# adria0/plonk-by-fingers

Measured on AMD Instinct MI355X. Metric: NTT elements/sec (Goldilocks, n=2^20 per GPU, natural order, bit-exact vs src/fft.rs), higher is better.
Workload: dtype u64 (Goldilocks p=2^64-2^32+1); 1 GPU; Goldilocks forward NTT, batch 32 x 2^20; n_per_gpu=1048576, n_global=1048576, batch=32, passes=default (2^20: 10,10)

## Files before the change

### plonk-by-fingers_amd/csrc/ntt_gl.hpp

```cpp
#pragma once
#include "ntt_kernels.hpp"

namespace pbf {

struct GlPassArgs {
  const uint64_t* in;
  uint64_t* out;
  const uint64_t* twpass;
  const uint64_t* tw0;
  const uint64_t* tw1;
  const uint64_t* tc;
  const uint64_t* tws_a;
  const uint64_t* tws_b;
  uint64_t n;
  uint32_t log_n;
  uint32_t log_ns;
  uint32_t tw_bits;
  uint32_t blocks_per_poly;
  uint32_t batch;
  uint32_t scaled;
  uint32_t out_split_log;
  uint32_t xcd_kmajor;
  uint64_t in_pitch, out_pitch;
  const uint64_t* post_tw;
  uint32_t skip_pass_tw;
  uint64_t blk_pitch;
  const uint64_t* cs_tab;
  const uint64_t* cs_tab1;
  uint32_t cs_bits;
  uint64_t cs_len;
};

__host__ __device__ constexpr bool gl_pow2_neg(int k) {
  const int raw = ((k % 192) + 192) % 192;
  return raw > 64 && raw <= 160;
}
template <int K>
__device__ __forceinline__ uint64_t gl_pow2_abs(uint64_t x) {
  constexpr int RAW = ((K % 192) + 192) % 192;
  if constexpr (RAW == 0) {
    return x;
  } else if constexpr (RAW > 160) {
    return gl_div_pow2<192 - RAW>(x);
  } else {
    using T = ShiftKind<RAW>;
    static_assert(T::NEG == gl_pow2_neg(K), "sign of 2^K");
    return apply_shift<Goldilocks, T>(x);
  }
}
template <int K>
__device__ __forceinline__ uint64_t gl_pow2(uint64_t x) {
  const uint64_t y = gl_pow2_abs<K>(x);
  if constexpr (gl_pow2_neg(K)) {
    const FieldArgs f{};
    return Goldilocks::sub(0, y, f);
  } else {
    return y;
  }
}

template <int E64, int Q1, int S2 = 1>
__device__ __forceinline__ void gl_stage_b_twiddle(uint64_t* v) {
  if constexpr (S2 < 16) {
    v[S2] = gl_pow2<(E64 * S2 * Q1) % 192>(v[S2]);
    gl_stage_b_twiddle<E64, Q1, S2 + 1>(v);
  }
}
template <int E64, int Q1, int S2 = 1>
__device__ __forceinline__ void gl_stage_b_twiddle_abs(uint64_t* v) {
  if constexpr (S2 < 16) {
    v[S2] = gl_pow2_abs<(E64 * S2 * Q1) % 192>(v[S2]);
    gl_stage_b_twiddle_abs<E64, Q1, S2 + 1>(v);
  }
}
__host__ __device__ constexpr unsigned gl_stage_b_negmask(int e64, int q1) {
  unsigned m = 0;
  for (int s2 = 1; s2 < 16; ++s2) m |= gl_pow2_neg((e64 * s2 * q1) % 192) ? 1u << s2 : 0u;
  return m;
}
constexpr int GL_B_LEVELS = 2;
template <int E64, int Q1>
__device__ __forceinline__ void gl_stage_b_head(uint64_t* v) {
  const FieldArgs f{};
  gl_stage_b_twiddle_abs<E64, Q1>(v);
  dft_reg_signed<Goldilocks, 4, sub_root_exp(E64, 4), gl_stage_b_negmask(E64, Q1), GL_B_LEVELS>(v, f);
}

template <int E64, int Q, int E = 1>
__device__ __forceinline__ void gl_post_twiddle_br(uint64_t* v) {
  if constexpr (E < 16) {
    v[bitrev_c(E, 4)] = gl_pow2<(E64 * E * Q) % 192>(v[bitrev_c(E, 4)]);
    gl_post_twiddle_br<E64, Q, E + 1>(v);
  }
}
template <int E64, int WV, int U = 0>
__device__ __forceinline__ void gl_rg3_c_shift(uint64_t* x) {
  if constexpr (U < 4) {
    constexpr int g = WV + 4 * U;
    x[U * 4 + 1] = gl_pow2<(E64 * g) % 192>(x[U * 4 + 1]);
    x[U * 4 + 2] = gl_pow2<(E64 * 2 * g) % 192>(x[U * 4 + 2]);
    x[U * 4 + 3] = gl_pow2<(E64 * 3 * g) % 192>(x[U * 4 + 3]);
    gl_rg3_c_shift<E64, WV, U + 1>(x);
  }
}

template <int LOGR, int TILE>
struct GlShape {
  static constexpr int R = 1 << LOGR;
  static constexpr int LOGC = LOGR - 6;
  static constexpr int C = 1 << LOGC;
  static constexpr int W = TILE / R;
  static constexpr int NT = TILE / 16;
  static constexpr int WPQ = NT / 256;
  static constexpr bool YX = W == 16 && C > 1;
  static constexpr int YP = (YX ? 64 : 65) * W;
  static constexpr int LDS = (C * YP > TILE) ? C * YP : TILE;
  static constexpr bool LDS32K = LDS * 8 <= 32768;
  static constexpr int NSUB_C = (64 * W) / NT;
  __host__ __device__ static constexpr int ysw(int k1) {
    return W <= 32 ? (k1 / (32 / W)) & (W - 1) : (k1 & 31);
  }
  __host__ __device__ static constexpr int yidx(int r2, int k1, int w) {
    return r2 * YP + (YX ? (k1 ^ (r2 & 1)) : k1) * W + (w ^ ysw(k1));
  }
};

__device__ __forceinline__ void gl_tile_coords(const GlPassArgs& a, uint32_t tile, uint32_t tiles, uint32_t* poly,
                                               uint32_t* kb) {
  if (a.xcd_kmajor == 1) {
    const uint32_t v = (tile & 7) * (tiles >> 3) + (tile >> 3);
    *kb = v / a.batch;
    *poly = v % a.batch;
  } else if (a.xcd_kmajor == 2) {
    const uint32_t v = (tile & 7) * (tiles >> 3) + (tile >> 3);
    *poly = v / a.blocks_per_poly;
    *kb = v % a.blocks_per_poly;
  } else {
    *poly = tile / a.blocks_per_poly;
    *kb = tile % a.blocks_per_poly;
  }
}

__device__ __forceinline__ uint64_t gl_cs_factor(const GlPassArgs& a, uint64_t i) {
  const FieldArgs f{};
  if (a.cs_tab1) return Goldilocks::mul(a.cs_tab[i & ((1ull << a.cs_bits) - 1)], a.cs_tab1[i >> a.cs_bits], f);
  return a.cs_tab[i];
}

constexpr int GL_STORES = 16;

constexpr uint64_t GL_BLK_PITCH = 8192;
static_assert(GL_BLK_PITCH >= 8192 && GL_BLK_PITCH % 2 == 0, "block pitch");
typedef uint64_t gl_u64x2 __attribute__((ext_vector_type(2)));

template <int LOGR, int E64, bool FIRST, int TILE, int RG = 0, int CS = 0, int SP = 0>
__device__ __forceinline__ void gl_tile(const GlPassArgs& a, uint64_t* lds, uint32_t tile, uint32_t tiles, int t) {
  using Sh = GlShape<LOGR, TILE>;
  constexpr int C = Sh::C, LOGC = Sh::LOGC, W = Sh::W, NT = Sh::NT, YP = Sh::YP;
  (void)YP;
  static_assert(Sh::NSUB_C * C == GL_STORES, "stores per thread");
  static_assert(SP == 0 || ((!FIRST || SP == 2) && RG == 0 && CS == 0 && SP <= 2), "SP: plain two-pass plan");
  static_assert(SP != 2 || (LOGR == 10 && TILE == 8192), "SP 2: the 10,10 plan");
  static_assert(RG == 0 || (LOGR == 8 && TILE == 4096 && FIRST == (RG == 1)), "RG shape");
  static_assert(CS == 0 || (FIRST == (CS == 1) && (RG == 0 || RG == 2 * CS - 1)), "CS 1: first pass, CS 2: last pass");
  const FieldArgs f{};
  using G = Goldilocks;
  uint32_t poly, kb;
  gl_tile_coords(a, tile, tiles, &poly, &kb);
  const uint64_t j0 = (uint64_t)kb * W;
  const uint64_t* in = a.in + (uint64_t)poly * a.in_pitch;
  const uint64_t stride = a.n >> LOGR;
  constexpr bool BLK_IN = SP == 2 && !FIRST, BLK_OUT = SP == 2 && FIRST;

  uint64_t v[16];
  if constexpr (BLK_IN) {
    const gl_u64x2* blk = (const gl_u64x2*)(in + (uint64_t)kb * a.blk_pitch) + t;
#pragma unroll
    for (int up = 0; up < 8; ++up) {
      const gl_u64x2 e = blk[512 * up];
      v[(2 * (up & 1)) * 4 + (up >> 1)] = e.x;
      v[(2 * (up & 1) + 1) * 4 + (up >> 1)] = e.y;
    }
  } else if constexpr (CS == 1) {
#pragma unroll
    for (int h = 0; h < 2; ++h) {
      uint64_t tw[8];
#pragma unroll
      for (int uu = 0; uu < 2; ++uu) {
        const int idx = t + NT * (2 * h + uu);
        const int w = idx % W, r2 = (idx / W) % C, s2 = idx / (C * W);
#pragma unroll
        for (int s1 = 0; s1 < 4; ++s1) {
          const uint64_t i = (j0 + w) + (uint64_t)(16 * C * s1 + C * s2 + r2) * stride;
          const bool on = i < a.cs_len;
          v[8 * h + uu * 4 + s1] = on ? in[i] : 0;
          tw[uu * 4 + s1] = on ? gl_cs_factor(a, i) : 0;
        }
      }
#pragma unroll
      for (int m = 0; m < 8; ++m) v[8 * h + m] = G::mul(v[8 * h + m], tw[m], f);
    }
  } else {
#pragma unroll
    for (int u = 0; u < 4; ++u) {
      const int idx = t + NT * u;
      const int w = idx % W, r2 = (idx / W) % C, s2 = idx / (C * W);
#pragma unroll
      for (int s1 = 0; s1 < 4; ++s1) {
        const int r = 16 * C * s1 + C * s2 + r2;
        v[u * 4 + s1] = in[(j0 + w) + (uint64_t)r * stride];
      }
    }
  }
  uint64_t t3[RG == 3 ? 2 : 1];
  if constexpr (RG == 3) {
    const int wave = t >> 6, q1 = wave / Sh::WPQ, rw = (wave % Sh::WPQ) * 64 + (t & 63);
    const int r2 = rw / W, w = rw % W;
    const uint64_t X = ((uint64_t)q1 << 16) + j0 + w;
    t3[0] = a.tws_a[((uint64_t)r2 << 18) + X];
    t3[1] = a.tws_b[X];
  }
  if constexpr (!FIRST && RG != 3 && SP == 0) if (!a.skip_pass_tw) {
    const uint64_t kmask = (1ull << a.log_ns) - 1;
#pragma unroll
    for (int h = 0; h < 2; ++h) {
      uint64_t tw[8];
#pragma unroll
      for (int uu = 0; uu < 2; ++uu) {
        const int u = 2 * h + uu;
        const int idx = t + NT * u;
        const int w = idx % W, r2 = (idx / W) % C, s2 = idx / (C * W);
        const uint64_t k = (j0 + w) & kmask;
#pragma unroll
        for (int s1 = 0; s1 < 4; ++s1) {
          const uint64_t r = (uint64_t)(16 * C * s1 + C * s2 + r2);
          if (a.twpass) {
            tw[uu * 4 + s1] = a.twpass[(r << a.log_ns) + k];
          } else if (a.tws_a) {
            tw[uu * 4 + s1] = G::mul(a.tws_b[(uint64_t)kb * Sh::R + r], a.tws_a[r * W + w], f);
          } else {
            const uint64_t e = ((r * k) << (a.log_n - a.log_ns - LOGR)) & (a.n - 1);
            tw[uu * 4 + s1] = G::mul(a.tw0[e & ((1ull << a.tw_bits) - 1)], a.tw1[e >> a.tw_bits], f);
          }
        }
      }
#pragma unroll
      for (int m = 0; m < 8; ++m) v[8 * h + m] = G::mul(v[8 * h + m], tw[m], f);
    }
  }
#pragma unroll
  for (int u = 0; u < 4; ++u) dft_reg<G, 2, sub_root_exp(E64, 2)>(v + u * 4, nullptr, f);
  if constexpr (BLK_IN) {
#pragma unroll
    for (int h = 0; h < 2; ++h) {
      const int s2 = 8 * h + (t >> 6);
#pragma unroll
      for (int q1 = 0; q1 < 4; ++q1) {
        gl_u64x2 e;
        e.x = v[(2 * h) * 4 + bitrev_c(q1, 2)];
        e.y = v[(2 * h + 1) * 4 + bitrev_c(q1, 2)];
        *(gl_u64x2*)(lds + (q1 * 16 + s2) * (C * W) + 2 * (t & 63)) = e;
      }
    }
  } else {
#pragma unroll
    for (int u = 0; u < 4; ++u) {
      const int idx = t + NT * u;
      const int s2 = idx / (C * W), rw = idx % (C * W);
#pragma unroll
      for (int q1 = 0; q1 < 4; ++q1) lds[(q1 * 16 + s2) * (C * W) + rw] = v[u * 4 + bitrev_c(q1, 2)];
    }
  }
  __syncthreads();

  {
    const int wave = t >> 6;
    const int q1 = wave / Sh::WPQ;
    const int rw = (wave % Sh::WPQ) * 64 + (t & 63);
#pragma unroll
    for (int s2 = 0; s2 < 16; ++s2) v[s2] = lds[(q1 * 16 + s2) * (C * W) + rw];
    if constexpr (RG == 3) {
      uint64_t p = t3[0];
      const uint64_t d = t3[1];
#pragma unroll
      for (int s2 = 0; s2 < 16; ++s2) {
        v[s2] = G::mul(v[s2], p, f);
        if (s2 < 15) p = G::mul(p, d, f);
      }
      dft_reg<G, 4, sub_root_exp(E64, 4)>(v, nullptr, f);
    } else {
      switch (__builtin_amdgcn_readfirstlane(q1)) {
        case 1: gl_stage_b_head<E64, 1>(v); break;
        case 2: gl_stage_b_head<E64, 2>(v); break;
        case 3: gl_stage_b_head<E64, 3>(v); break;
        default: gl_stage_b_head<E64, 0>(v); break;
      }
      dft_reg_tail<G, 4, sub_root_exp(E64, 4), GL_B_LEVELS>(v, f);
    }
    __syncthreads();
    const int r2 = rw / W, w = rw % W;
#pragma unroll
    for (int q2 = 0; q2 < 16; ++q2) {
      const int k1 = q1 + 4 * q2;
      lds[Sh::yidx(r2, k1, w)] = v[bitrev_c(q2, 4)];
    }
  }
  __syncthreads();

  auto c_map = [&](int u, int* k1, int* w) {
    const int idx = t + NT * u;
    if constexpr (BLK_OUT) {
      *k1 = 8 * (t >> 6) + (t & 7);
      *w = (t >> 3) & 7;
    } else if constexpr (FIRST) {
      *k1 = idx & 63;
      *w = idx >> 6;
    } else {
      *k1 = idx / W;
      *w = idx % W;
    }
  };
  uint64_t x[Sh::NSUB_C * C];
#pragma unroll
  for (int u = 0; u < Sh::NSUB_C; ++u) {
    int k1, w;
    c_map(u, &k1, &w);
#pragma unroll
    for (int r2 = 0; r2 < C; ++r2) x[u * C + r2] = lds[Sh::yidx(r2, k1, w)];
  }
  if constexpr (RG == 3) {
    switch (__builtin_amdgcn_readfirstlane(t >> 6)) {
      case 0: gl_rg3_c_shift<E64, 0>(x); break;
      case 1: gl_rg3_c_shift<E64, 1>(x); break;
      case 2: gl_rg3_c_shift<E64, 2>(x); break;
      default: gl_rg3_c_shift<E64, 3>(x); break;
    }
  } else if constexpr (RG == 1) {
    const uint64_t* tc = a.tc + ((j0 >> 12) & 15) * 256;
#pragma unroll
    for (int u = 0; u < Sh::NSUB_C; ++u) {
      int k1, w;
      c_map(u, &k1, &w);
      uint64_t tw[C];
#pragma unroll
      for (int r2 = 0; r2 < C; ++r2) tw[r2] = tc[r2 * 64 + k1];
#pragma unroll
      for (int r2 = 0; r2 < C; ++r2) x[u * C + r2] = G::mul(x[u * C + r2], tw[r2], f);
    }
  } else {
    uint64_t tw[Sh::NSUB_C * C];
    const bool scaled = SP == 0 && a.scaled;
    const int r2lo = scaled ? 0 : 1;
#pragma unroll
    for (int u = 0; u < Sh::NSUB_C; ++u) {
      int k1, w;
      c_map(u, &k1, &w);
#pragma unroll
      for (int r2 = 0; r2 < C; ++r2) tw[u * C + r2] = (r2 >= r2lo) ? a.tc[r2 * 64 + k1] : 1;
    }
    if (scaled) {
#pragma unroll
      for (int m = 0; m < Sh::NSUB_C * C; ++m) x[m] = G::mul(x[m], tw[m], f);
    } else {
#pragma unroll
      for (int u = 0; u < Sh::NSUB_C; ++u)
#pragma unroll
        for (int r2 = 1; r2 < C; ++r2) x[u * C + r2] = G::mul(x[u * C + r2], tw[u * C + r2], f);
    }
  }
  if constexpr (C > 1) {
#pragma unroll
    for (int u = 0; u < Sh::NSUB_C; ++u) dft_reg<G, LOGC, sub_root_exp(E64, LOGC)>(x + u * C, nullptr, f);
  }

  if constexpr (BLK_OUT) {
    static_assert(Sh::NSUB_C == 1 && W == 8, "tile-major stores: one sub-DFT per thread");
    const uint64_t base = (uint64_t)__builtin_amdgcn_readfirstlane(t >> 6) * a.blk_pitch + j0 * W;
    const uint32_t lane = t & 63;
    const uint64_t* ptw = a.post_tw + base;
    uint64_t* o = a.out + (uint64_t)poly * a.out_pitch + base;
    uint64_t tw[C];
#pragma unroll
    for (int k2 = 0; k2 < C; ++k2) tw[k2] = ptw[(uint64_t)(8 * k2) * a.blk_pitch + lane];
#pragma unroll
    for (int k2 = 0; k2 < C; ++k2) x[bitrev_c(k2, LOGC)] = G::mul(x[bitrev_c(k2, LOGC)], tw[k2], f);
#pragma unroll
    for (int k2 = 0; k2 < C; ++k2) o[(uint64_t)(8 * k2) * a.blk_pitch + lane] = x[bitrev_c(k2, LOGC)];
  } else if constexpr (FIRST) {
    uint64_t* o = a.out + (uint64_t)poly * a.out_pitch;
#pragma unroll
    for (int u = 0; u < Sh::NSUB_C; ++u) {
      int k1, w;
      c_map(u, &k1, &w);
      const uint64_t base = (j0 + w) << LOGR;
      if (a.post_tw) {
        uint64_t tw[C];
#pragma unroll
        for (int k2 = 0; k2 < C; ++k2) tw[k2] = a.post_tw[base + k1 + 64 * k2];
#pragma unroll
        for (int k2 = 0; k2 < C; ++k2) x[u * C + bitrev_c(k2, LOGC)] = G::mul(x[u * C + bitrev_c(k2, LOGC)], tw[k2], f);
      }
#pragma unroll
      for (int k2 = 0; k2 < C; ++k2) o[base + k1 + 64 * k2] = x[u * C + bitrev_c(k2, LOGC)];
    }
  } else {
    const uint32_t lns = SP == 2 ? (uint32_t)LOGR : a.log_ns;
    const uint64_t ns_mask = (1ull << lns) - 1;
    uint64_t* out = a.out + (uint64_t)poly * a.out_pitch;
    const uint32_t sl = SP != 0 ? 0u : a.out_split_log;
#pragma unroll
    for (int u = 0; u < Sh::NSUB_C; ++u) {
      int k1, w;
      c_map(u, &k1, &w);
      const uint64_t j = j0 + w;
      const uint64_t base = ((j >> lns) << (lns + LOGR)) + (j & ns_mask);
      if (sl == 0) {
        if constexpr (CS == 2) {
          uint64_t tw[C];
#pragma unroll
          for (int k2 = 0; k2 < C; ++k2) tw[k2] = gl_cs_factor(a, base + ((uint64_t)(k1 + 64 * k2) << lns));
#pragma unroll
          for (int k2 = 0; k2 < C; ++k2) x[u * C + bitrev_c(k2, LOGC)] = G::mul(x[u * C + bitrev_c(k2, LOGC)], tw[k2], f);
        }
#pragma unroll
        for (int k2 = 0; k2 < C; ++k2) out[base + ((uint64_t)(k1 + 64 * k2) << lns)] = x[u * C + bitrev_c(k2, LOGC)];
      } else {
        const uint64_t smask = (1ull << sl) - 1;
#pragma unroll
        for (int k2 = 0; k2 < C; ++k2) {
          const uint64_t kk = base + ((uint64_t)(k1 + 64 * k2) << lns);
          a.out[((((kk >> sl) * a.batch) + poly) << sl) + (kk & smask)] = x[u * C + bitrev_c(k2, LOGC)];
        }
      }
    }
  }
}

template <int LOGR, int TILE>
__device__ __forceinline__ void gl_shape_checks() {
  using Sh = GlShape<LOGR, TILE>;
  static_assert(LOGR >= 6 && LOGR <= 10, "radix 2^6 .. 2^10");
  static_assert(Sh::LDS * 8 <= (TILE > 8192 ? 160 : 80) * 1024, "LDS budget");
  static_assert(Sh::W >= 8 && Sh::WPQ >= 1, "tile shape");
}

template <int LOGR, int E64, bool FIRST, int TILE, int RG = 0, int CS = 0, int SP = 0>
__global__ void __launch_bounds__(TILE / 16)
__attribute__((amdgpu_waves_per_eu((FIRST || RG) && GlShape<LOGR, TILE>::LDS32K ? 5 : 4)))
ntt_gl_pass_kernel(GlPassArgs a) {
  gl_shape_checks<LOGR, TILE>();
  __shared__ __attribute__((aligned(16))) uint64_t lds[GlShape<LOGR, TILE>::LDS];
  const uint32_t tiles = a.blocks_per_poly * a.batch;
  gl_tile<LOGR, E64, FIRST, TILE, RG, CS, SP>(a, lds, blockIdx.x, tiles, threadIdx.x);
}

template <int E64>
__global__ void __launch_bounds__(256) __attribute__((amdgpu_waves_per_eu(4))) ntt_gl_rg2_kernel(GlPassArgs a) {
  constexpr int W = 16;
  __shared__ __attribute__((aligned(16))) uint64_t lds[16 * 16 * W];
  const FieldArgs f{};
  using G = Goldilocks;
  const uint32_t tiles = a.blocks_per_poly * a.batch;
  uint32_t poly, kb;
  gl_tile_coords(a, blockIdx.x, tiles, &poly, &kb);
  const int t = threadIdx.x, w = t % W, a1h = t / W;
  const uint64_t j0 = (uint64_t)kb * W, j = j0 + w;
  const uint32_t c = (uint32_t)(j0 >> 6) & 3, a1l = (uint32_t)(j0 >> 14) & 3;
  const uint64_t* in = a.in + (uint64_t)poly * a.in_pitch;
  const uint64_t stride = a.n >> 8;
  uint64_t v[16], tw[16];
#pragma unroll
  for (int a2l = 0; a2l < 16; ++a2l) v[a2l] = in[j + (uint64_t)(a2l * 16 + a1h) * stride];
  const uint64_t* t2 = a.twpass + ((uint64_t)(a1l + 4 * a1h) << 12) + (j & 255);
#pragma unroll
  for (int d = 0; d < 16; ++d) tw[d] = t2[256 * d];
  switch (__builtin_amdgcn_readfirstlane(c)) {
    case 1: gl_stage_b_twiddle<E64, 1>(v); break;
    case 2: gl_stage_b_twiddle<E64, 2>(v); break;
    case 3: gl_stage_b_twiddle<E64, 3>(v); break;
    default: break;
  }
  dft_reg<G, 4, sub_root_exp(E64, 4)>(v, nullptr, f);
#pragma unroll
  for (int d = 0; d < 16; ++d) lds[d * 256 + (a1h ^ (d & 3)) * W + w] = G::mul(v[bitrev_c(d, 4)], tw[d], f);
  __syncthreads();
  const int d2 = t / W;
#pragma unroll
  for (int h = 0; h < 16; ++h) v[h] = lds[d2 * 256 + (h ^ (d2 & 3)) * W + w];
  dft_reg<G, 4, sub_root_exp(E64, 4)>(v, nullptr, f);
  switch (__builtin_amdgcn_readfirstlane(a1l)) {
    case 1: gl_post_twiddle_br<E64, 1>(v); break;
    case 2: gl_post_twiddle_br<E64, 2>(v); break;
    case 3: gl_post_twiddle_br<E64, 3>(v); break;
    default: break;
  }
  uint64_t* out = a.out + (uint64_t)poly * a.out_pitch;
  const uint64_t base = ((j >> 8) << 16) + (j & 255);
#pragma unroll
  for (int e = 0; e < 16; ++e) out[base + ((uint64_t)(d2 + 16 * e) << 8)] = v[bitrev_c(e, 4)];
}

}
```

### plonk-by-fingers_amd/csrc/ntt_launch.hip

```cpp
#include <cstdlib>
#include <cstring>
#include <mutex>
#include "internal.hpp"
#include "ntt_gl.hpp"

namespace pbf {

bool hinv(uint64_t a, uint64_t m, uint64_t* out) {
  __int128 s = 0, old_s = 1, r = m, old_r = a % m;
  while (r != 0) {
    __int128 q = old_r / r, t;
    t = old_r - q * r; old_r = r; r = t;
    t = old_s - q * s; old_s = s; s = t;
  }
  if (old_r != 1) return false;
  if (old_s < 0) old_s += m;
  *out = (uint64_t)old_s;
  return true;
}

bool field_for(uint64_t m, FieldKind* kind, FieldArgs* fa) {
  fa->m = m;
  fa->mu = 0;
  if (m == GOLDILOCKS) { *kind = FIELD_GOLDILOCKS; return true; }
// ... 241 lines not shown
  if (rc) return rc;
  if ((rc = run_plan_impl(p, d_in, (uint64_t*)s2.p, batch, s0, s1, stream, 0))) return rc;
  hipLaunchKernelGGL(shard_split_kernel, dim3(grid_for(p.n * batch)), dim3(256), 0, stream, (const uint64_t*)s2.p,
                     d_send, S, p.n, (uint32_t)batch);
  PBF_HIP(hipGetLastError());
  return 0;
}

int launch_shard_unsplit(const uint64_t* recv, uint64_t* out, uint64_t nl, uint32_t batch, uint32_t G,
                         hipStream_t s) {
  hipLaunchKernelGGL(shard_unsplit_kernel, dim3(grid_for(nl * batch)), dim3(256), 0, s, recv, out, nl / G, nl, batch,
                     G);
  PBF_HIP(hipGetLastError());
  return 0;
}

int make_two_level(uint64_t m, uint64_t root, uint64_t n, TwoLevel* t) {
  uint32_t log_n = 0;
  while ((1ull << log_n) < n) ++log_n;
  t->bits = (log_n + 1) / 2;
  t->root = root;
  const auto tw = two_level_tabs(root, n, t->bits, 1, m);
  int rc = upload(t->t0, tw.first);
  return rc ? rc : upload(t->t1, tw.second);
}

template <class F>
static int combine_typed(const FieldArgs& fa, const TwoLevel& tl, uint32_t G, uint64_t rank, const uint64_t* in,
                         uint64_t* out, uint64_t nl, uint32_t batch, int inverse, hipStream_t s) {
  CombineArgs a;
  a.recv = in; a.out = out;
  a.tw0 = (const uint64_t*)tl.t0.p; a.tw1 = (const uint64_t*)tl.t1.p; a.tw_bits = tl.bits;
  a.nl = nl; a.s = nl / G; a.rank = rank; a.n_mask = (uint64_t)G * nl - 1; a.batch = batch; a.f = fa;
  a.scale = 1;
  if (inverse) {
    uint64_t ginv;
    if (!hinv(G % fa.m, fa.m, &ginv)) return fail(2, "G has no inverse");
    a.scale = ginv;
  }
  for (int i = 0; i < 8; ++i) a.wg[i] = 0;
  const uint64_t wG = hpow(tl.root, nl, fa.m);
  uint64_t x = 1 % fa.m;
  for (uint32_t i = 0; i < G; ++i) { a.wg[i] = x; x = hmul(x, wG, fa.m); }
  const uint64_t total = (nl / G) * batch;
  void (*fn)(CombineArgs) = nullptr;
  switch (G) {
    case 2: fn = inverse ? shard_split_inv_kernel<F, 2> : shard_combine_kernel<F, 2>; break;
    case 4: fn = inverse ? shard_split_inv_kernel<F, 4> : shard_combine_kernel<F, 4>; break;
    case 8: fn = inverse ? shard_split_inv_kernel<F, 8> : shard_combine_kernel<F, 8>; break;
    default: return fail(1, "world size must be 2, 4 or 8");
  }
  hipLaunchKernelGGL(fn, dim3(grid_for(total)), dim3(256), 0, s, a);
  PBF_HIP(hipGetLastError());
  return 0;
}

int launch_shard_combine(FieldKind k, const FieldArgs& fa, const TwoLevel& tl, uint32_t G, uint64_t rank,
                         const uint64_t* in, uint64_t* out, uint64_t nl, uint32_t batch, int inverse, hipStream_t s) {
  return with_field(k, [&](auto F) {
    return combine_typed<decltype(F)>(fa, tl, G, rank, in, out, nl, batch, inverse, s);
  });
}

typedef void (*GlPassFn)(GlPassArgs);

struct GlPassDesc {
  int logr;
  bool first;
  int rg;
  int cs;
  int sp;
};

static bool two_pass_tw(const NttPlan& p, uint32_t split_log) {
  return p.logr.size() == 2 && split_log == 0 && p.twpass[1]->p;
}

static bool gl_blocked(const NttPlan& p, bool coset, uint32_t split_log) {
  return two_pass_tw(p, split_log) && !coset && p.post_blk.p != nullptr;
}

static uint64_t gl_scratch_pitch(const NttPlan& p, bool coset, uint32_t split_log) {
  return gl_blocked(p, coset, split_log) ? 128 * GL_BLK_PITCH : p.n;
}

static GlPassDesc gl_pass_desc(const NttPlan& p, size_t i, bool coset, uint32_t split_log) {
  const size_t P = p.logr.size();
  GlPassDesc d{p.logr[i], i == 0, 0, 0, 0};
  if (p.rg && P == 3 && split_log == 0) d.rg = (int)i + 1;
  if (coset && !p.inverse && i == 0) d.cs = 1;
  if (coset && p.inverse && i == P - 1) d.cs = 2;
  if (gl_blocked(p, coset, split_log)) d.sp = 2;
  else if (two_pass_tw(p, split_log) && i == 1 && !coset && !p.inverse && p.e64 == 39 && d.logr == 10) d.sp = 1;
  return d;
}

template <int E, int LR>
static GlPassFn gl_kernel_lr(const GlPassDesc& d) {
  constexpr int T = gl_tile(LR);
  if (d.first) return d.cs ? ntt_gl_pass_kernel<LR, E, true, T, 0, 1> : ntt_gl_pass_kernel<LR, E, true, T>;
  return d.cs ? ntt_gl_pass_kernel<LR, E, false, T, 0, 2> : ntt_gl_pass_kernel<LR, E, false, T>;
}

template <int E>
static GlPassFn gl_kernel_e(const GlPassDesc& d) {
  if (d.rg == 1) return d.cs ? ntt_gl_pass_kernel<8, E, true, 4096, 1, 1> : ntt_gl_pass_kernel<8, E, true, 4096, 1>;
  if (d.rg == 2) return ntt_gl_rg2_kernel<E>;
  if (d.rg == 3) return d.cs ? ntt_gl_pass_kernel<8, E, false, 4096, 3, 2> : ntt_gl_pass_kernel<8, E, false, 4096, 3>;
  if constexpr (E == 39) {
    if (d.sp == 1) return ntt_gl_pass_kernel<10, E, false, 8192, 0, 0, 1>;
    if (d.sp == 2) return d.first ? ntt_gl_pass_kernel<10, E, true, 8192, 0, 0, 2> : ntt_gl_pass_kernel<10, E, false, 8192, 0, 0, 2>;
  }
  switch (d.logr) {
    case 6: return gl_kernel_lr<E, 6>(d);
    case 7: return gl_kernel_lr<E, 7>(d);
    case 8: return gl_kernel_lr<E, 8>(d);
    case 9: return gl_kernel_lr<E, 9>(d);
    case 10: return gl_kernel_lr<E, 10>(d);
    default: return nullptr;
  }
}

static GlPassFn gl_kernel(const GlPassDesc& d, int e64) {
  return e64 == 39 ? gl_kernel_e<39>(d) : gl_kernel_e<153>(d);
}

static int run_gl_group(const NttPlan& p, const uint64_t* d_in, uint64_t* d_out, size_t batch, DevBuf& s0,
                        DevBuf& s1, hipStream_t stream, uint32_t split_log, size_t soff = 0,
                        const GlCoset* cs = nullptr);

int ForkSet::ensure(int streams) {
  if (streams > GL_MAX_STREAMS) streams = GL_MAX_STREAMS;
  const unsigned flags = hipEventDisableTiming | hipEventDisableSystemFence;
  if (streams > 1 && !fork) PBF_HIP(hipEventCreateWithFlags(&fork, flags));
  for (int i = 1; i < streams; ++i) {
    if (!aux[i]) PBF_HIP(hipStreamCreateWithFlags(&aux[i], hipStreamNonBlocking));
    if (!join[i]) PBF_HIP(hipEventCreateWithFlags(&join[i], flags));
  }
  return 0;
}

ForkSet::~ForkSet() {
  (void)hipSetDevice(device);
  for (int i = 1; i < GL_MAX_STREAMS; ++i) {
    if (aux[i]) {
      (void)hipStreamSynchronize(aux[i]);
      (void)hipStreamDestroy(aux[i]);
    }
    if (join[i]) (void)hipEventDestroy(join[i]);
  }
  if (fork) (void)hipEventDestroy(fork);
}

static void gl_schedule(const NttPlan& p, size_t batch, uint32_t split_log, const ForkSet* fork, size_t* G, int* ns) {
  const long long go = p.opts.num("ntt.group", -1);
  *G = go >= 0 ? (size_t)go : (batch >= 8 ? 4 : batch);
  if (split_log != 0 || *G >= batch) *G = 0;
  *ns = (int)p.opts.num("ntt.streams", 2);
  *ns = *ns < 1 ? 1 : (*ns > GL_MAX_STREAMS ? GL_MAX_STREAMS : *ns);
  if (!fork || *G == 0) *ns = 1;
}

static size_t gl_scratch_polys(const NttPlan& p, size_t batch, uint32_t split_log, const ForkSet* fork) {
  size_t G;
  int ns;
  gl_schedule(p, batch, split_log, fork, &G, &ns);
  return (G == 0 || G * ns > batch) ? batch : G * ns;
}

static int run_gl_passes(const NttPlan& p, const uint64_t* d_in, uint64_t* d_out, size_t batch, DevBuf& s0,
                         DevBuf& s1, hipStream_t stream, uint32_t split_log, ForkSet* fork, const GlCoset* cs) {
  size_t G;
  int ns;
  gl_schedule(p, batch, split_log, fork, &G, &ns);
  if (G == 0) return run_gl_group(p, d_in, d_out, batch, s0, s1, stream, split_log, 0, cs);
  const size_t in_pitch = (cs && !p.inverse) ? cs->in_len : p.n;
  hipStream_t sts[GL_MAX_STREAMS];
  sts[0] = stream;
  if (ns > 1) {
    int rc = fork->ensure(ns);
    if (rc) return rc;
    for (int i = 1; i < ns; ++i) sts[i] = fork->aux[i];
    PBF_HIP(hipEventRecord(fork->fork, stream));
    for (int i = 1; i < ns; ++i) PBF_HIP(hipStreamWaitEvent(sts[i], fork->fork, 0));
  }
  int gi = 0;
  for (size_t g0 = 0; g0 < batch; g0 += G, ++gi) {
    const size_t b = batch - g0 < G ? batch - g0 : G;
    const int rc = run_gl_group(p, d_in + g0 * in_pitch, d_out + g0 * p.n, b, s0, s1, sts[gi % ns], 0,
                                (size_t)(gi % ns) * G * gl_scratch_pitch(p, cs != nullptr, split_log), cs);
    if (rc) return rc;
  }
  for (int i = 1; i < ns; ++i) {
    PBF_HIP(hipEventRecord(fork->join[i], sts[i]));
    PBF_HIP(hipStreamWaitEvent(stream, fork->join[i], 0));
  }
  return 0;
}

static int ensure_rg_tables(const NttPlan& p) {
  if (p.rg_built) return 0;
  const uint64_t m = p.m, n = p.n;
  const uint64_t w = p.root;
  int rc;
  const uint64_t w4096 = hpow(w, n / 4096, m);
  std::vector<uint64_t> tc1(4096);
  for (uint64_t a2l = 0; a2l < 16; ++a2l)
    for (uint64_t r2 = 0; r2 < 4; ++r2)
      for (uint64_t k1 = 0; k1 < 64; ++k1)
        tc1[a2l * 256 + r2 * 64 + k1] = hpow(w4096, ((a2l + 16 * r2) * k1) % 4096, m);
  const Table t2 = pass_tab(hpow(w, 64, m), 64, 4096, m);
  const uint64_t scale = p.inverse ? p.n_inv : 1;
  std::vector<uint64_t> tgc(4ull << 18), tgb(1ull << 18);
  {
    const uint64_t w4 = hpow(w, 4, m);
    uint64_t x1 = 1, x4 = 1;
    for (uint64_t X = 0; X < (1ull << 18); ++X) {
      tgb[X] = x4;
      uint64_t c = scale;
      for (uint64_t r2 = 0; r2 < 4; ++r2) {
        tgc[(r2 << 18) + X] = c;
        c = hmul(c, x1, m);
      }
      x1 = hmul(x1, w, m);
      x4 = hmul(x4, w4, m);
    }
  }
  if ((rc = upload(p.rg_tc1, tc1)) || (rc = upload(p.rg_t2, t2)) || (rc = upload(p.rg_tgc, tgc)) ||
      (rc = upload(p.rg_tgb, tgb)))
    return rc;
  p.rg_built = true;
  return 0;
}

static GlPassArgs gl_pass_args(const NttPlan& p, size_t i, const GlPassDesc& d, uint32_t log_ns, const uint64_t* in,
                               uint64_t* out, size_t batch, uint32_t split_log, const GlCoset* cs) {
  const bool last = i == p.logr.size() - 1;
  const uint64_t W = (uint64_t)gl_tile(d.logr) >> d.logr;
  GlPassArgs a;
  a.in = in;
  a.out = out;
  a.in_pitch = a.out_pitch = p.n;
  a.twpass = (const uint64_t*)p.twpass[i]->p;
  a.tw0 = (const uint64_t*)p.tw0.p;
  a.tw1 = (const uint64_t*)p.tw1.p;
  a.tc = (const uint64_t*)p.tc[i]->p;
  const bool tws = !a.twpass && last && p.tws_a && (uint64_t)p.tws_w == W;
  a.tws_a = tws ? (const uint64_t*)p.tws_a->p : nullptr;
  a.tws_b = tws ? (const uint64_t*)p.tws_b->p : nullptr;
  a.n = p.n;
  a.log_n = p.log_n;
  a.log_ns = log_ns;
  a.tw_bits = p.tw_bits;
  a.blocks_per_poly = (uint32_t)((p.n >> d.logr) / W);
  a.batch = (uint32_t)batch;
  a.scaled = (p.inverse && last) ? 1 : 0;
  a.out_split_log = last ? split_log : 0;
  const uint64_t tiles = (uint64_t)a.blocks_per_poly * batch;
  a.xcd_kmajor = (log_ns > 0 && batch > 1 && tiles % 8 == 0) ? 1 : 0;
  a.post_tw = nullptr;
  a.skip_pass_tw = 0;
  if (two_pass_tw(p, split_log)) {
    if (i == 0) a.post_tw = (const uint64_t*)p.twpass[1]->p;
    else a.skip_pass_tw = 1;
  }
  if (a.post_tw && batch > 1 && tiles % 8 == 0) a.xcd_kmajor = 1;
  a.blk_pitch = 0;
  if (d.sp == 2) {
    a.blk_pitch = GL_BLK_PITCH;
    if (i == 0) {
      a.post_tw = (const uint64_t*)p.post_blk.p;
      a.out_pitch = 128 * GL_BLK_PITCH;
    } else {
      a.in_pitch = 128 * GL_BLK_PITCH;
      a.xcd_kmajor = 0;
    }
  }
  a.cs_tab = a.cs_tab1 = nullptr;
  a.cs_bits = 0;
  a.cs_len = 0;
  if (d.cs) {
    a.cs_tab = (const uint64_t*)cs->tabs->t0.p;
    a.cs_tab1 = (const uint64_t*)cs->tabs->t1.p;
    a.cs_bits = cs->tabs->bits;
    if (d.cs == 1) {
      a.cs_len = cs->in_len;
      a.in_pitch = cs->in_len;
    } else if (!d.rg) {
      a.tc = (const uint64_t*)cs->tabs->tc_last.p;
      a.scaled = 0;
    }
  }
  if (d.rg) {
    if (d.rg == 1) a.tc = (const uint64_t*)p.rg_tc1.p;
    if (d.rg == 2) a.twpass = (const uint64_t*)p.rg_t2.p;
    if (d.rg == 3) {
      a.twpass = nullptr;
      a.tws_a = (const uint64_t*)p.rg_tgc.p;
      a.tws_b = (const uint64_t*)p.rg_tgb.p;
    }
    if (tiles % 8 == 0) a.xcd_kmajor = 2;
  }
  return a;
}

static int run_gl_group(const NttPlan& p, const uint64_t* d_in, uint64_t* d_out, size_t batch, DevBuf& s0,
                        DevBuf& s1, hipStream_t stream, uint32_t split_log, size_t soff, const GlCoset* cs) {
  const size_t P = p.logr.size();
  if (cs && (split_log != 0 || P < 2)) return fail(1, "coset transform: unsupported plan");
  if (gl_pass_desc(p, 0, cs != nullptr, split_log).rg) {
    const int rc = ensure_rg_tables(p);
    if (rc) return rc;
  }
  uint32_t log_ns = 0;
  for (size_t i = 0; i < P; ++i) {
    const GlPassDesc d = gl_pass_desc(p, i, cs != nullptr, split_log);
    const GlPassFn fn = gl_kernel(d, p.e64);
    if (!fn) return fail(1, "no Goldilocks pass kernel for this radix");
    const int tile = gl_tile(d.logr);
    if ((p.n >> d.logr) % (tile >> d.logr)) return fail(1, "transform too small for the pass tile");
    const uint64_t* in = (i == 0) ? d_in : (const uint64_t*)(((i - 1) & 1) ? s1.p : s0.p) + soff;
    uint64_t* out = (i == P - 1) ? d_out : (uint64_t*)((i & 1) ? s1.p : s0.p) + soff;
    const GlPassArgs a = gl_pass_args(p, i, d, log_ns, in, out, batch, split_log, cs);
    const uint64_t tiles = (uint64_t)a.blocks_per_poly * batch;
    if (tiles > 0x7fffffffull) return fail(1, "batch too large");
    hipLaunchKernelGGL(fn, dim3((uint32_t)tiles), dim3(tile / 16), 0, stream, a);
    PBF_HIP(hipGetLastError());
    log_ns += d.logr;
  }
  return 0;
}

static int run_plan_impl(const NttPlan& p, const uint64_t* d_in, uint64_t* d_out, size_t batch, DevBuf& s0,
                         DevBuf& s1, hipStream_t stream, uint32_t split_log, ForkSet* fork, const GlCoset* cs) {
  if (batch == 0) return 0;
  if (p.n == 1) {
    if (d_in != d_out) PBF_HIP(hipMemcpyAsync(d_out, d_in, batch * 8, hipMemcpyDeviceToDevice, stream));
    return 0;
  }
  if (p.logr.empty()) {
    with_field(p.kind, [&](auto F) {
      hipLaunchKernelGGL(ntt_small_kernel<decltype(F)>, dim3(batch), dim3(256), 0, stream, d_in, d_out,
                         (const uint64_t*)p.small_tw.p, p.log_n, p.n_inv, (uint32_t)p.inverse, p.fa);
    });
    PBF_HIP(hipGetLastError());
    return 0;
  }
  const size_t P = p.logr.size();
  const size_t bytes = p.gl ? gl_scratch_polys(p, batch, split_log, fork) * gl_scratch_pitch(p, cs != nullptr, split_log) * 8
                            : batch * p.n * 8;
  int rc = s0.ensure(bytes);
  if (!rc && P > 2) rc = s1.ensure(bytes);
  if (rc) return rc;
  uint32_t log_ns = 0;
  if (p.gl) return run_gl_passes(p, d_in, d_out, batch, s0, s1, stream, split_log, fork, cs);
  if (cs) return fail(1, "coset transform: not a Goldilocks standard-root plan");
  for (size_t i = 0; i < P; ++i) {
    const int lr = p.logr[i];
    const PassFn fn = pass_fn(p.kind, p.e64, lr);
    if (!fn) return fail(1, "no kernel for this radix");
    const int W = cols_for(lr);
    PassArgs a;
    a.in = (i == 0) ? d_in : (const uint64_t*)(((i - 1) & 1) ? s1.p : s0.p);
    a.out = (i == P - 1) ? d_out : (uint64_t*)((i & 1) ? s1.p : s0.p);
    a.tw0 = (const uint64_t*)p.tw0.p;
    a.tw1 = (const uint64_t*)p.tw1.p;
    a.rtab = (const uint64_t*)p.rtab[i]->p;
    a.twpass = (const uint64_t*)p.twpass[i]->p;
    a.n = p.n;
    a.n_inv = p.n_inv;
    a.log_n = p.log_n;
    a.log_ns = log_ns;
    a.tw_bits = p.tw_bits;
    a.blocks_per_poly = (uint32_t)((p.n >> lr) / W);
    a.scale = (p.inverse && i == P - 1) ? 1 : 0;
    a.out_split_log = (i == P - 1) ? split_log : 0;
    a.batch = (uint32_t)batch;
    a.f = p.fa;
    const int nt = (W << lr) >> NTT_LQ;
    const uint64_t blocks = (uint64_t)a.blocks_per_poly * batch;
    if (blocks > 0x7fffffffull) return fail(1, "batch too large");
    const uint32_t grid = (uint32_t)blocks;
    a.xcd_kmajor = (log_ns > 0 && batch > 1 && grid % 8 == 0) ? 1 : 0;
    hipLaunchKernelGGL(fn, dim3(grid), dim3(nt), 0, stream, a);
    PBF_HIP(hipGetLastError());
    log_ns += lr;
  }
  return 0;
}

static uint32_t log2_ceil(uint64_t x) {
  uint32_t l = 0;
  while ((1ull << l) < x) ++l;
  return l;
}

static int coset_tabs(const NttPlan& p, uint64_t shift, uint64_t len, const CosetTabs** out) {
  const uint64_t m = p.m;
  CosetTabs* t = nullptr;
  for (auto& c : p.coset)
    if (c->shift == shift) t = c.get();
  if (t && t->len >= len) {
    t->stamp = ++p.coset_clock;
    *out = t;
    return 0;
  }
  if (!t) {
    if (p.coset.size() >= COSET_SHIFTS_PER_PLAN) {
      size_t old = 0;
      for (size_t i = 1; i < p.coset.size(); ++i)
        if (p.coset[i]->stamp < p.coset[old]->stamp) old = i;
      p.coset.erase(p.coset.begin() + old);
    }
    p.coset.emplace_back(new CosetTabs());
    t = p.coset.back().get();
    t->shift = shift;
  } else {
    PBF_HIP(hipDeviceSynchronize());
  }
  t->len = 0;
  uint64_t s = shift, c = 1 % m;
  if (p.inverse) {
    if (!hinv(shift, m, &s)) return fail(1, "shift has no inverse");
    if (p.gl && !p.rg) c = p.n_inv;
  }
  int rc;
  if (len <= (1ull << p.twmax_log)) {
    t->bits = 0;
    t->t1.release();
    if ((rc = upload(t->t0, geometric(c, s, len, m)))) return rc;
  } else {
    t->bits = (log2_ceil(len) + 1) / 2;
    const auto tw = two_level_tabs(s, len, t->bits, c, m);
    if ((rc = upload(t->t0, tw.first)) || (rc = upload(t->t1, tw.second))) return rc;
  }
  if (p.gl && !p.rg && p.inverse && !t->tc_last.p) {
    const uint64_t R = 1ull << p.logr.back();
    if ((rc = upload(t->tc_last, stage_c_tab(hpow(p.root, p.n / R, m), R / 64, 1, m)))) return rc;
  }
  t->len = len;
  t->stamp = ++p.coset_clock;
  *out = t;
  return 0;
}

template <class F>
__global__ void coset_scale_kernel(const uint64_t* in, uint64_t in_len, uint64_t* out, uint64_t n, uint64_t batch,
                                   const uint64_t* t0, const uint64_t* t1, uint32_t bits, FieldArgs f) {
  const uint64_t total = n * batch;
  for (uint64_t id = (uint64_t)blockIdx.x * blockDim.x + threadIdx.x; id < total;
       id += (uint64_t)gridDim.x * blockDim.x) {
    const uint64_t b = id / n, i = id % n;
    uint64_t y = 0;
    if (i < in_len) {
      const uint64_t tw = t1 ? F::mul(t0[i & ((1ull << bits) - 1)], t1[i >> bits], f) : t0[i];
      y = F::mul(in[b * in_len + i], tw, f);
    }
    out[id] = y;
  }
}

static int launch_coset_scale(const NttPlan& p, const CosetTabs& t, const uint64_t* in, uint64_t in_len, uint64_t* out,
                              uint64_t batch, hipStream_t s) {
  const dim3 grid((uint32_t)grid_for(p.n * batch));
  with_field(p.kind, [&](auto F) {
    hipLaunchKernelGGL(coset_scale_kernel<decltype(F)>, grid, dim3(256), 0, s, in, in_len, out, p.n, batch,
                       (const uint64_t*)t.t0.p, (const uint64_t*)t.t1.p, t.bits, p.fa);
  });
  PBF_HIP(hipGetLastError());
  return 0;
}

int run_plan_coset(const NttPlan& p, uint64_t shift, const uint64_t* d_in, size_t in_len, uint64_t* d_out,
                   size_t batch, DevBuf& s0, DevBuf& s1, hipStream_t stream, ForkSet* fork) {
  if (batch == 0) return 0;
  if (p.n == 1 || (shift == 1 && in_len == p.n)) return run_plan_impl(p, d_in, d_out, batch, s0, s1, stream, 0, fork);
  const CosetTabs* t;
  int rc = coset_tabs(p, shift, p.inverse ? p.n : in_len, &t);
  if (rc) return rc;
  if (p.gl) {
    const GlCoset cs{t, in_len};
    return run_plan_impl(p, d_in, d_out, batch, s0, s1, stream, 0, fork, &cs);
  }
  if (p.inverse) {
    if ((rc = run_plan_impl(p, d_in, d_out, batch, s0, s1, stream, 0, fork))) return rc;
    return launch_coset_scale(p, *t, d_out, p.n, d_out, batch, stream);
  }
  if ((rc = launch_coset_scale(p, *t, d_in, in_len, d_out, batch, stream))) return rc;
  return run_plan_impl(p, d_out, d_out, batch, s0, s1, stream, 0, fork);
}

int launch_pointwise_mul(FieldKind k, const FieldArgs& fa, const uint64_t* a, const uint64_t* b, uint64_t* c,
                         uint64_t count, hipStream_t s) {
  uint64_t blocks = (count + 255) / 256;
  if (blocks > 4096) blocks = 4096;
  if (blocks == 0) return 0;
  with_field(k, [&](auto F) {
    hipLaunchKernelGGL(pointwise_mul_kernel<decltype(F)>, dim3(blocks), dim3(256), 0, s, a, b, c, count, fa);
  });
  PBF_HIP(hipGetLastError());
  return 0;
}
// ... 95 lines not shown
```

Baseline: 112.4 billion elements/s.

## Exchange 64-bit values through LDS in 32-bit halves to fit three workgroups per CU

For the 10,10 blocked plan, the in-tile LDS transposes now move the low and high 32-bit halves of each value in two rounds. This halves the LDS buffer so three workgroups fit per CU, and waves_per_eu is raised to 6. The reads are hand-written ds_read_b32 inline asm with fixed strides. The cost is extra barriers and twice as many LDS instructions. Separately, the default batch group size goes from 4 to 8 for blocked plans when the batch is at least 16.

```diff
diff --git a/plonk-by-fingers_amd/csrc/ntt_gl.hpp b/plonk-by-fingers_amd/csrc/ntt_gl.hpp
--- a/plonk-by-fingers_amd/csrc/ntt_gl.hpp
+++ b/plonk-by-fingers_amd/csrc/ntt_gl.hpp
@@ -149,6 +149,35 @@
 
 constexpr int GL_STORES = 16;
 
+__host__ __device__ constexpr bool gl_split(int sp) { return sp == 2; }
+typedef uint32_t gl_u32x2 __attribute__((ext_vector_type(2)));
+#define GL_RD(i, off) "ds_read_b32 %" #i ", %16 offset:" #off "\n\t"
+template <int STRIDE>
+__device__ __forceinline__ void gl_lds_read16(const uint32_t* p, uint32_t* o) {
+  static_assert(STRIDE == 512 || STRIDE == 2080, "the strides written out below: Z (C*W words), Y (YP words)");
+  const uint32_t a = (uint32_t)(uintptr_t)(const __attribute__((address_space(3))) uint32_t*)p;
+#define GL_RD_OUT                                                                                                   \
+  "=&v"(o[0]), "=&v"(o[1]), "=&v"(o[2]), "=&v"(o[3]), "=&v"(o[4]), "=&v"(o[5]), "=&v"(o[6]), "=&v"(o[7]), "=&v"(o[8]), \
+      "=&v"(o[9]), "=&v"(o[10]), "=&v"(o[11]), "=&v"(o[12]), "=&v"(o[13]), "=&v"(o[14]), "=&v"(o[15])
+  if constexpr (STRIDE == 512) {
+    asm volatile(GL_RD(0, 0) GL_RD(1, 512) GL_RD(2, 1024) GL_RD(3, 1536) GL_RD(4, 2048) GL_RD(5, 2560) GL_RD(6, 3072)
+                     GL_RD(7, 3584) GL_RD(8, 4096) GL_RD(9, 4608) GL_RD(10, 5120) GL_RD(11, 5632) GL_RD(12, 6144)
+                         GL_RD(13, 6656) GL_RD(14, 7168) GL_RD(15, 7680) "s_waitcnt lgkmcnt(0)"
+                 : GL_RD_OUT
+                 : "v"(a)
+                 : "memory");
+  } else {
+    asm volatile(GL_RD(0, 0) GL_RD(1, 2080) GL_RD(2, 4160) GL_RD(3, 6240) GL_RD(4, 8320) GL_RD(5, 10400) GL_RD(6, 12480)
+                     GL_RD(7, 14560) GL_RD(8, 16640) GL_RD(9, 18720) GL_RD(10, 20800) GL_RD(11, 22880) GL_RD(12, 24960)
+                         GL_RD(13, 27040) GL_RD(14, 29120) GL_RD(15, 31200) "s_waitcnt lgkmcnt(0)"
+                 : GL_RD_OUT
+                 : "v"(a)
+                 : "memory");
+  }
+#undef GL_RD_OUT
+}
+#undef GL_RD
+
 constexpr uint64_t GL_BLK_PITCH = 8192;
 static_assert(GL_BLK_PITCH >= 8192 && GL_BLK_PITCH % 2 == 0, "block pitch");
 typedef uint64_t gl_u64x2 __attribute__((ext_vector_type(2)));
@@ -171,6 +200,9 @@
   const uint64_t* in = a.in + (uint64_t)poly * a.in_pitch;
   const uint64_t stride = a.n >> LOGR;
   constexpr bool BLK_IN = SP == 2 && !FIRST, BLK_OUT = SP == 2 && FIRST;
+  constexpr bool SPLIT = gl_split(SP);
+  uint32_t* lds32 = (uint32_t*)lds;
+  (void)lds32;
 
   uint64_t v[16];
   if constexpr (BLK_IN) {
@@ -250,7 +282,46 @@
   }
 #pragma unroll
   for (int u = 0; u < 4; ++u) dft_reg<G, 2, sub_root_exp(E64, 2)>(v + u * 4, nullptr, f);
-  if constexpr (BLK_IN) {
+  if constexpr (SPLIT) {
+    const int q1r = (t >> 6) / Sh::WPQ, rwr = ((t >> 6) % Sh::WPQ) * 64 + (t & 63);
+    uint32_t zl[16];
+#pragma unroll
+    for (int hw = 0; hw < 2; ++hw) {
+      if (hw) __syncthreads();
+      if constexpr (BLK_IN) {
+#pragma unroll
+        for (int h = 0; h < 2; ++h) {
+          const int s2 = 8 * h + (t >> 6);
+#pragma unroll
+          for (int q1 = 0; q1 < 4; ++q1) {
+            gl_u32x2 e;
+            e.x = (uint32_t)(v[(2 * h) * 4 + bitrev_c(q1, 2)] >> (32 * hw));
+            e.y = (uint32_t)(v[(2 * h + 1) * 4 + bitrev_c(q1, 2)] >> (32 * hw));
+            *(gl_u32x2*)(lds32 + (q1 * 16 + s2) * (C * W) + 2 * (t & 63)) = e;
+          }
+        }
+      } else {
+#pragma unroll
+        for (int u = 0; u < 4; ++u) {
+          const int idx = t + NT * u;
+          const int s2 = idx / (C * W), rw = idx % (C * W);
+#pragma unroll
+          for (int q1 = 0; q1 < 4; ++q1)
+            lds32[(q1 * 16 + s2) * (C * W) + rw] = (uint32_t)(v[u * 4 + bitrev_c(q1, 2)] >> (32 * hw));
+        }
+      }
+      __syncthreads();
+      static_assert(C * W * 4 == 512, "Z stride of gl_lds_read16");
+      if (hw == 0) {
+        gl_lds_read16<512>(lds32 + q1r * 16 * (C * W) + rwr, zl);
+      } else {
+        uint32_t zh[16];
+        gl_lds_read16<512>(lds32 + q1r * 16 * (C * W) + rwr, zh);
+#pragma unroll
+        for (int s2 = 0; s2 < 16; ++s2) v[s2] = ((uint64_t)zh[s2] << 32) | zl[s2];
+      }
+    }
+  } else if constexpr (BLK_IN) {
 #pragma unroll
     for (int h = 0; h < 2; ++h) {
       const int s2 = 8 * h + (t >> 6);
@@ -271,14 +342,25 @@
       for (int q1 = 0; q1 < 4; ++q1) lds[(q1 * 16 + s2) * (C * W) + rw] = v[u * 4 + bitrev_c(q1, 2)];
     }
   }
-  __syncthreads();
-
+  if constexpr (!SPLIT) __syncthreads();
+
+  int tc = t;
+  auto y_write_half = [&](int hw) {
+    const int wv = tc >> 6, q1 = wv / Sh::WPQ, rw = (wv % Sh::WPQ) * 64 + (tc & 63);
+    const int r2 = rw / W, w = rw % W;
+    static_assert(!SPLIT || (W == 8 && Sh::yidx(3, 2 + 4 * 13, 6) == 3 * YP + 2 * W + (6 ^ (13 & 7)) + 4 * W * 13), "Y address form");
+#pragma unroll
+    for (int q2 = 0; q2 < 16; ++q2)
+      lds32[(r2 * YP + q1 * W + (w ^ (q2 & 7))) + 4 * W * q2] = (uint32_t)(v[bitrev_c(q2, 4)] >> (32 * hw));
+  };
   {
     const int wave = t >> 6;
     const int q1 = wave / Sh::WPQ;
     const int rw = (wave % Sh::WPQ) * 64 + (t & 63);
-#pragma unroll
-    for (int s2 = 0; s2 < 16; ++s2) v[s2] = lds[(q1 * 16 + s2) * (C * W) + rw];
+    if constexpr (!SPLIT) {
+#pragma unroll
+      for (int s2 = 0; s2 < 16; ++s2) v[s2] = lds[(q1 * 16 + s2) * (C * W) + rw];
+    }
     if constexpr (RG == 3) {
       uint64_t p = t3[0];
       const uint64_t d = t3[1];
@@ -297,12 +379,20 @@
       }
       dft_reg_tail<G, 4, sub_root_exp(E64, 4), GL_B_LEVELS>(v, f);
     }
+    if constexpr (SPLIT) {
+      asm volatile("" : "+v"(tc));
+      __builtin_assume(tc >= 0 && tc < NT);
+    }
     __syncthreads();
-    const int r2 = rw / W, w = rw % W;
-#pragma unroll
-    for (int q2 = 0; q2 < 16; ++q2) {
-      const int k1 = q1 + 4 * q2;
-      lds[Sh::yidx(r2, k1, w)] = v[bitrev_c(q2, 4)];
+    if constexpr (SPLIT) {
+      y_write_half(0);
+    } else {
+      const int r2 = rw / W, w = rw % W;
+#pragma unroll
+      for (int q2 = 0; q2 < 16; ++q2) {
+        const int k1 = q1 + 4 * q2;
+        lds[Sh::yidx(r2, k1, w)] = v[bitrev_c(q2, 4)];
+      }
     }
   }
   __syncthreads();
@@ -310,11 +400,14 @@
   auto c_map = [&](int u, int* k1, int* w) {
     const int idx = t + NT * u;
     if constexpr (BLK_OUT) {
-      *k1 = 8 * (t >> 6) + (t & 7);
-      *w = (t >> 3) & 7;
+      *k1 = 8 * (tc >> 6) + (tc & 7);
+      *w = (tc >> 3) & 7;
     } else if constexpr (FIRST) {
       *k1 = idx & 63;
       *w = idx >> 6;
+    } else if constexpr (SPLIT) {
+      *k1 = tc / W;
+      *w = tc % W;
     } else {
       *k1 = idx / W;
       *w = idx % W;
@@ -325,8 +418,21 @@
   for (int u = 0; u < Sh::NSUB_C; ++u) {
     int k1, w;
     c_map(u, &k1, &w);
-#pragma unroll
-    for (int r2 = 0; r2 < C; ++r2) x[u * C + r2] = lds[Sh::yidx(r2, k1, w)];
+    if constexpr (SPLIT) {
+      static_assert(Sh::NSUB_C == 1, "split exchange: one sub-DFT per thread");
+      static_assert(C == 16 && YP * 4 == 2080, "Y stride of gl_lds_read16");
+      uint32_t yl[C], yh[C];
+      gl_lds_read16<2080>(lds32 + Sh::yidx(0, k1, w), yl);
+      __syncthreads();
+      y_write_half(1);
+      __syncthreads();
+      gl_lds_read16<2080>(lds32 + Sh::yidx(0, k1, w), yh);
+#pragma unroll
+      for (int r2 = 0; r2 < C; ++r2) x[r2] = ((uint64_t)yh[r2] << 32) | yl[r2];
+    } else {
+#pragma unroll
+      for (int r2 = 0; r2 < C; ++r2) x[u * C + r2] = lds[Sh::yidx(r2, k1, w)];
+    }
   }
   if constexpr (RG == 3) {
     switch (__builtin_amdgcn_readfirstlane(t >> 6)) {
@@ -375,8 +481,8 @@
 
   if constexpr (BLK_OUT) {
     static_assert(Sh::NSUB_C == 1 && W == 8, "tile-major stores: one sub-DFT per thread");
-    const uint64_t base = (uint64_t)__builtin_amdgcn_readfirstlane(t >> 6) * a.blk_pitch + j0 * W;
-    const uint32_t lane = t & 63;
+    const uint64_t base = (uint64_t)__builtin_amdgcn_readfirstlane(tc >> 6) * a.blk_pitch + j0 * W;
+    const uint32_t lane = tc & 63;
     const uint64_t* ptw = a.post_tw + base;
     uint64_t* o = a.out + (uint64_t)poly * a.out_pitch + base;
     uint64_t tw[C];
@@ -446,10 +552,12 @@
 
 template <int LOGR, int E64, bool FIRST, int TILE, int RG = 0, int CS = 0, int SP = 0>
 __global__ void __launch_bounds__(TILE / 16)
-__attribute__((amdgpu_waves_per_eu((FIRST || RG) && GlShape<LOGR, TILE>::LDS32K ? 5 : 4)))
+__attribute__((amdgpu_waves_per_eu(gl_split(SP) ? 6 : (FIRST || RG) && GlShape<LOGR, TILE>::LDS32K ? 5 : 4)))
 ntt_gl_pass_kernel(GlPassArgs a) {
   gl_shape_checks<LOGR, TILE>();
-  __shared__ __attribute__((aligned(16))) uint64_t lds[GlShape<LOGR, TILE>::LDS];
+  constexpr int LDS64 = GlShape<LOGR, TILE>::LDS / (gl_split(SP) ? 2 : 1);
+  static_assert(!gl_split(SP) || 3 * LDS64 * 8 <= 160 * 1024, "split exchange: three workgroups per CU");
+  __shared__ __attribute__((aligned(16))) uint64_t lds[LDS64];
   const uint32_t tiles = a.blocks_per_poly * a.batch;
   gl_tile<LOGR, E64, FIRST, TILE, RG, CS, SP>(a, lds, blockIdx.x, tiles, threadIdx.x);
 }
diff --git a/plonk-by-fingers_amd/csrc/ntt_launch.hip b/plonk-by-fingers_amd/csrc/ntt_launch.hip
--- a/plonk-by-fingers_amd/csrc/ntt_launch.hip
+++ b/plonk-by-fingers_amd/csrc/ntt_launch.hip
@@ -417,19 +417,21 @@
   if (fork) (void)hipEventDestroy(fork);
 }
 
-static void gl_schedule(const NttPlan& p, size_t batch, uint32_t split_log, const ForkSet* fork, size_t* G, int* ns) {
+static void gl_schedule(const NttPlan& p, size_t batch, bool coset, uint32_t split_log, const ForkSet* fork, size_t* G,
+                        int* ns) {
   const long long go = p.opts.num("ntt.group", -1);
-  *G = go >= 0 ? (size_t)go : (batch >= 8 ? 4 : batch);
+  const size_t dflt = gl_blocked(p, coset, split_log) && batch >= 16 ? 8 : 4;
+  *G = go >= 0 ? (size_t)go : (batch >= 8 ? dflt : batch);
   if (split_log != 0 || *G >= batch) *G = 0;
   *ns = (int)p.opts.num("ntt.streams", 2);
   *ns = *ns < 1 ? 1 : (*ns > GL_MAX_STREAMS ? GL_MAX_STREAMS : *ns);
   if (!fork || *G == 0) *ns = 1;
 }
 
-static size_t gl_scratch_polys(const NttPlan& p, size_t batch, uint32_t split_log, const ForkSet* fork) {
+static size_t gl_scratch_polys(const NttPlan& p, size_t batch, bool coset, uint32_t split_log, const ForkSet* fork) {
   size_t G;
   int ns;
-  gl_schedule(p, batch, split_log, fork, &G, &ns);
+  gl_schedule(p, batch, coset, split_log, fork, &G, &ns);
   return (G == 0 || G * ns > batch) ? batch : G * ns;
 }
 
@@ -437,7 +439,7 @@
                          DevBuf& s1, hipStream_t stream, uint32_t split_log, ForkSet* fork, const GlCoset* cs) {
   size_t G;
   int ns;
-  gl_schedule(p, batch, split_log, fork, &G, &ns);
+  gl_schedule(p, batch, cs != nullptr, split_log, fork, &G, &ns);
   if (G == 0) return run_gl_group(p, d_in, d_out, batch, s0, s1, stream, split_log, 0, cs);
   const size_t in_pitch = (cs && !p.inverse) ? cs->in_len : p.n;
   hipStream_t sts[GL_MAX_STREAMS];
@@ -612,7 +614,7 @@
     return 0;
   }
   const size_t P = p.logr.size();
-  const size_t bytes = p.gl ? gl_scratch_polys(p, batch, split_log, fork) * gl_scratch_pitch(p, cs != nullptr, split_log) * 8
+  const size_t bytes = p.gl ? gl_scratch_polys(p, batch, cs != nullptr, split_log, fork) * gl_scratch_pitch(p, cs != nullptr, split_log) * 8
                             : batch * p.n * 8;
   int rc = s0.ensure(bytes);
   if (!rc && P > 2) rc = s1.ensure(bytes);
```

After: 124.0 billion elements/s (median of 6 runs). +10.4%, better.
